# johnnyjana730/MVIN

Hardware: AMD Instinct MI355X
Metric: (user,item) pairs scored/sec @ dim=64 hop=2 fan-out=32; % HBM roofline (higher is better)
Workload: dtype f32

## Files before the change

### mvin_amd/csrc/mvin_kernels.h

```cpp
#pragma once
#include <hip/hip_runtime.h>
#include <stdint.h>

#include "../../include/mvin_hip.h"
#include "mvin_common.h"

namespace mvin {

struct GatherAttnArgs {
    int gather;
    int table_bf16;
    const void* table;
    const int32_t* adj_e;
    const int32_t* adj_r;
    const int32_t* node_ids;
    const float* neigh;
    const int32_t* rel_ids;
    const float* rel_score;
    const float* self_vec;
    const float* Wc;
    const float* c_child;
    const float* Wagg;
    const float* bagg;
    float* out;
    float* probs;
    float* s_out;
    float* z_out;
    int64_t T;
    int N, K, D, lpr_log2;
    int tile_rows;
};

struct RippleArgs {
    const void* E;
    int table_bf16;
    const int32_t* score_ids;
    const int32_t* rel_ids;
    const int32_t* value_ids;
    const float* V;
    const float* w;
    float* out;
    int64_t ldo;
    int64_t B;
    int mode, Nm, D, nR, lpr_log2;
};

struct RippleBuildArgs {
    const int64_t* indptr;
    const int32_t* dst;
    const int32_t* rel;
    const int64_t* hist_ptr;
    const int32_t* hist_items;
    int32_t* out;
    int64_t n_user;
    uint64_t seed;
    int P, Nm, n_neighbor;
};

struct KeyAddrArgs {
    const void* E;
    const float* V;
    const float* w;
    const int32_t* mem_h[8];
    const int32_t* mem_r[8];
    const int32_t* mem_t[8];
    float* out;
    int64_t ldo;
    int64_t B;
    int P, Nm, D, nR, lpr_log2;
    uint64_t table_bytes;
    const int32_t* uts;
    const int64_t* users64;
    const int32_t* users32;
    int n_user;
    int n_entity;
};

struct KeyAddrLists {
    const int32_t *h, *r, *t;
};
__device__ __forceinline__ KeyAddrLists key_addr_lists(const KeyAddrArgs& a, int64_t b, int hop) {
    if (a.uts) {
        int64_t u = a.users64 ? a.users64[b] : (int64_t)a.users32[b];
        u = u < 0 ? 0 : (u >= a.n_user ? a.n_user - 1 : u);
        const int32_t* base = a.uts + ((u * (a.P > 0 ? a.P : 1) + hop) * 3) * (int64_t)a.Nm;
        return {base, base + a.Nm, base + 2 * a.Nm};
    }
    const int64_t o = b * a.Nm;
    return {a.mem_h[hop] + o, hop < a.P ? a.mem_r[hop] + o : nullptr, hop < a.P ? a.mem_t[hop] + o : nullptr};
}

struct KeyAddrGroupedArgs {
    const void* E;
    const float* R;
    const float* w;
    const int32_t* uts;
    const int32_t* seg_user;
    const int32_t* seg_ptr;
    const int32_t* nseg_dev;
    const int32_t* pair_index;
    const int64_t* items64;
    const int32_t* items32;
    float* out;
    int64_t ldo;
    int nseg, P, Nm, D, nR, NRL;
    int n_entity;
    int dbg;
    const int32_t* records;
    const float* ER;
    const float* hs;
};

struct KaFlashArgs {
    const float* E;
    const float* ER;
    const float* hs;
    const int32_t* records;
    const int32_t* seg_user;
    const int32_t* seg_ptr;
    const int32_t* nseg_dev;
    const int32_t* pair_index;
    const int64_t* items64;
    const int32_t* items32;
    const float* TW;
    const float* bmlp;
    float* user_o;
    int32_t* slot_seg;
    int32_t* counter;
    int nslots;
    int P, Nm, nR, n_entity;
    int64_t B;
};

struct KaRecLayout {
    int NmP, rows, maxtiles, o_cnt, o_off, o_trel, o_bidx, o_head, o_tail, o_hr, len;
};

struct TailArgs {
    const void* E;
    const int64_t* items64;
    const int32_t* items32;
    const float* q;
    const float* user_o;
    const float* nagg0;
    const float* nagg1;
    const float* W0;
    const float* b0;
    const float* A0;
    const float* a0;
    const float* A1;
    const float* a1;
    const float* Wmix;
    const float* bmix;
    float* item_emb;
    float* scores;
    float* sig;
    int64_t B;
    int table_bf16;
    int n_entity;
    int dbg;
};

struct EntityAggArgs {
    const float* tabS;
    const float* tabG;
    const float* selfS;
    const float* selfG;
    const int32_t* adj_e;
    const int32_t* adj_r;
    const float* t0;
    float* outS;
    float* outG;
    int n_entity, K, nR;
    uint64_t table_bytes, adj_bytes;
    int D;
};

struct TailFoldArgs {
    const float* M0;
    const int64_t* items64;
    const int32_t* items32;
    const float* q;
    const float* user_o;
    const float* out0;
    const float* z2;
    const float* Wqm;
    const float* A1;
    const float* a1;
    const float* Wmix;
    const float* bm;
    float* item_emb;
    float* scores;
    float* sig;
    int64_t B;
    int n_entity;
};

struct GatherMixArgs {
    const void* table;
    const int32_t* adj_e;
    const int32_t* adj_r;
    const int32_t* node_ids;
    const float* rel_score;
    const float* rowbias;
    float* out;
    int64_t nodes;
    int npg, K, D, lpr_log2, relu, table_bf16;
};

struct FusedL2Args {
    const void* table;
    const int32_t* adj_e;
    const int32_t* adj_r;
    const int32_t* parent_ids;
    const float* t0;
    const float* t1;
    const float* W1;
    const float* W2;
    const float* q;
    const float* b1;
    const float* b2;
    const float* A0;
    const float* a0;
    float* nagg0;
    float* nagg1;
    float* probs_parent;
    float* probs_child;
    int64_t P;
    uint64_t table_bytes;
    uint64_t adj_bytes;
    int parents_per_pair, K, nR, lpn_log2;
    int pid_stride;
    unsigned max_id;
    int dbg;
    const int32_t* order;
    float* agg;
    int fold;
    int prj;
};

__device__ __forceinline__ int fused_parent_id(const FusedL2Args& a, int64_t i) {
    const unsigned v = (unsigned)a.parent_ids[i * a.pid_stride];
    return (int)(v < a.max_id ? v : a.max_id);
}

struct EltArgs {
    int mode;
    int64_t n;
    float* x;
    float* y;
    float* z;
    float* w;
    float* accum;
    float alpha, beta, beta1, beta2, eps;
    int D, N;
};

struct WgradArgs {
    mvin_linear_args lin;
    const float* dY;
    int64_t ldy, dy_zstride;
    const float* mask;
    int64_t ldm, mask_zstride;
    float* dW;
    int64_t dw_zstride;
    float* db;
    int64_t db_zstride;
    int IB;
};

struct AggBwdArgs {
    int gather;
    const float* table;
    const int32_t* adj_e;
    const int32_t* adj_r;
    const int32_t* node_ids;
    const float* child;
    const int32_t* rel_ids;
    const float* probs;
    const float* rel_score;
    int skip_zero;
    const float* dvec;
    float* dtable;
    float* dchild;
    float* dT;
    int64_t T;
    int K, D, nR, lpr_log2;
};

struct KeyAddrBwdArgs {
    KeyAddrArgs f;
    const float* dout;
    float* dE;
    float* dV;
    float* dw;
    float l2;
    const float* Rk;
    const void* items;
    int items64;
    int dw_rep;
    int dv_lds;
    float* reg_accum;
};

hipError_t launch_eltwise(const EltArgs& a, hipStream_t st);
hipError_t launch_l2_adam_multi(const mvin_param_seg* segs, int nseg, int64_t total, float* g, float* mo, float* vo,
                                float* accum, int apply_adam, float lr_t, const float* lr_dev, float b1, float b2,
                                float eps, hipStream_t st);
hipError_t launch_scatter_add_rows(float* dtable, const int32_t* ids, int ids64, const float* x, int64_t rows, int D,
                                   float alpha, hipStream_t st);
hipError_t launch_linear_wgrad(WgradArgs a, hipStream_t st);
hipError_t launch_linear_wgrad_multi(const WgradArgs* probs, int n, hipStream_t st);
hipError_t launch_agg_bwd(const AggBwdArgs& a, hipStream_t st);
hipError_t launch_rel_score_bwd(const float* rel, const float* urh_w, const float* dT, int nR, int D, float* drel,
                                float* durh, hipStream_t st);
hipError_t launch_key_addr_bwd(const KeyAddrBwdArgs& a, hipStream_t st);

inline int lpr_log2_for(int D) {
    int l = 0;
    while ((4 << l) < D) ++l;
    return l;
}

hipError_t launch_expand(const int32_t* adj_e, const int32_t* adj_r, const int64_t* items64,
                         const int32_t* items32, int B, int K, int levels, int n_entity,
                         int32_t* ent_out, int32_t* rel_out, hipStream_t st);
hipError_t launch_rel_score(const float* rel, const float* urh_w, int nR, int D, float* t,
                            hipStream_t st);
hipError_t launch_linear(const mvin_linear_args& a, hipStream_t st);
bool linear_mfma_supported(const mvin_linear_args& a);
hipError_t launch_linear_mfma(const mvin_linear_args& a, hipStream_t st);
hipError_t launch_gather_attn(const GatherAttnArgs& a, hipStream_t st);
hipError_t launch_ripple(const RippleArgs& a, hipStream_t st);
hipError_t launch_sample_adjacency(const int64_t* indptr, const int32_t* dst, const int32_t* rel, int n_entity,
                                   int K, uint64_t seed, int32_t* adj_e, int32_t* adj_r, hipStream_t st);
hipError_t launch_ripple_build(const RippleBuildArgs& a, hipStream_t st);
int key_addr_nj(int Nm, int D);
bool key_addr_grouped_supported(int D, int P, int Nm, int nR);
hipError_t launch_key_addr_grouped(const KeyAddrGroupedArgs& a, int table_bf16, hipStream_t st);
bool key_addr_wave16_supported(int D, int P, int Nm, int nR);
bool key_addr_wave16_applies(const KeyAddrGroupedArgs& a);
hipError_t launch_key_addr_wave16(const KeyAddrGroupedArgs& a, int table_bf16, hipStream_t st);
bool key_addr_dense_supported(int D, int P, int Nm, int nR);
hipError_t launch_key_addr_dense(const KeyAddrGroupedArgs& a, int table_bf16, hipStream_t st);
KaRecLayout ka_rec_layout(int P, int Nm, int nR);
hipError_t launch_user_records(const int32_t* uts, int n_user, int P, int Nm, int nR, int n_entity, int32_t* out, hipStream_t st);
bool key_addr_static_supported(int D, int P, int Nm, int nR);
bool key_addr_static_applies(const KeyAddrGroupedArgs& a, int table_bf16);
hipError_t launch_key_addr_static(const KeyAddrGroupedArgs& a, hipStream_t st);
bool key_addr_flash_supported(int D, int P, int Nm, int nR, int n_entity);
size_t key_addr_flash_ws_elems(int64_t B, int nseg_bound);
hipError_t launch_key_addr_flash(const KaFlashArgs& a, int nseg_bound, bool has_set, int32_t* sched_ws, hipStream_t st);
hipError_t kas_read_trace(long long* host_dst, size_t n);
hipError_t kaf_read_trace(long long* host_dst, size_t n);
hipError_t launch_key_addr(const KeyAddrArgs& a, int table_bf16, hipStream_t st);
bool key_addr_stream_supported(const KeyAddrArgs& a, int table_bf16);
hipError_t launch_key_addr_stream(const KeyAddrArgs& a, int table_bf16, hipStream_t st);
hipError_t launch_move_rows(void* table, const int32_t* ids, int64_t n, int row_bytes, void* rows, bool scatter,
                            hipStream_t st);
hipError_t launch_shard_space_ids(const void* ids, bool is64, int64_t n, int world, int n_local, void* out, hipStream_t st);
hipError_t launch_row_softmax(const float* x, int64_t rows, int n, float* out, hipStream_t st);
hipError_t launch_mix_urv(const float* neigh, const float* rel, const float* user, const float* logits, int64_t nodes, int N, int K,
                          int D, float* out, float* probs, hipStream_t st);
hipError_t launch_gather_mix(const GatherMixArgs& a, hipStream_t st);
struct ScoreSmallArgs {
    const void* E;
    const int32_t* adj_e;
    const int32_t* adj_r;
    const float* R;
    const float* w_h;
    const float* Wu;
    const float* bu;
    const float* t0;
    const float* t1;
    const float *W0, *b0, *W1, *b1, *W2, *b2;
    const float *A0, *a0, *A1, *a1, *Wmix, *bmix;
    const int64_t* items;
    const int32_t* mem_h[4];
    const int32_t* mem_r[4];
    const int32_t* mem_t[4];
    const int32_t* uts;
    const int64_t* users;
    float* user_o;
    float* item_emb;
    float* scores;
    float* sig;
    int64_t B;
    int G;
    int K, P, Nm, nR, n_entity, n_user, enc, table_bf16;
    int depth1;
    int dbg;
    uint64_t table_bytes;
    uint64_t adj_bytes;
};
bool score_small_supported(int D, int K, int P, int Nm, int nR);
int score_small_group(int D, int K, int P, int Nm, int nR, int has_hset, int64_t B);
hipError_t launch_score_small(ScoreSmallArgs a, int D, hipStream_t st);
hipError_t small_read_trace(long long* host_dst, size_t n);

bool l2_tail_supported(int D);
hipError_t launch_l2_tail(const TailArgs& a, int D, hipStream_t st);
bool l2_tail_flash_applies(const TailArgs& a, int D);
hipError_t launch_l2_tail_flash(const TailArgs& a, hipStream_t st);
bool fused_l2_supported(int D, int K);
hipError_t launch_gather_attn_l2(const FusedL2Args& a, int D, int table_bf16, hipStream_t st);
bool fused_split_supported(int D, int K);
bool fused_split_applies(const FusedL2Args& a, int D);
hipError_t launch_gather_probe_l2(const void* table, const int32_t* ids1, const int32_t* ids2, int64_t n_parents, int K,
                                  int D, int table_bf16, float* sums, hipStream_t st);
hipError_t launch_group_pairs(const int64_t* u64, const int32_t* u32, int64_t B, int n_user, int32_t* count, int32_t* offs,
                              int32_t* rank, int32_t* seg_user, int32_t* seg_ptr, int32_t* nseg, int32_t* pair_index, hipStream_t st);
hipError_t launch_count_ids(const int32_t* ids, int64_t n, int nbins, float* out, hipStream_t st);
bool fused_d32_supported(int D, int K);
bool fused_d32_applies(const FusedL2Args& a, int D);
size_t order_ws_elems(int64_t B);
hipError_t launch_order_by_key(const int64_t* k64, const int32_t* k32, int64_t B, int32_t* ws, int32_t* order, hipStream_t st);
bool fused_wpp_supported(int D, int K);
bool fused_wpp_applies(const FusedL2Args& a, int D);
hipError_t launch_gather_attn_l2_wpp(const FusedL2Args& a, hipStream_t st);
bool fused_agg_supported(int D, int K);
bool fused_fold_supported(int D, int K);
size_t fused_fold_lds_bytes(int D, int nR, int K);
bool fused_agg_applies(const FusedL2Args& a, int D);
hipError_t launch_entity_aggregates(const EntityAggArgs& a, hipStream_t st);
hipError_t launch_fold_prepare(const float* W0, const float* b0, const float* W1, const float* b1, const float* W2, const float* b2, const float* A0,
                               const float* a0, const float* Wmix, const float* bmix, const float* A1, float c, int D, float* blk, hipStream_t st);
hipError_t launch_l2_tail_fold(const TailFoldArgs& a, hipStream_t st);
hipError_t launch_score_l2_folded(const float* agg, const float* M0, const int32_t* adj_e, const int32_t* adj_r, const int32_t* items, int pid_stride,
                                  const float* t1, const float* q, const float* user_o, const float* Wq, const float* bq, const float* Wv,
                                  const float* bv, const float* Wqm, const float* A1, const float* a1, const float* Wm1, const float* Wm2,
                                  const float* bm, float* item_emb, float* scores, float* sig, int64_t B, int K, int D, int nR, int n_entity,
                                  hipStream_t st);
hipError_t launch_gather_attn_l2_agg(const FusedL2Args& a, hipStream_t st);
hipError_t launch_gather_attn_l2_d32(const FusedL2Args& a, int table_bf16, hipStream_t st, bool encoded = false);
bool fused_d16_supported(int D, int K);
bool fused_d16_applies(const FusedL2Args& a, int D);
hipError_t launch_gather_attn_l2_d16(const FusedL2Args& a, int table_bf16, hipStream_t st);
bool fused_l2_split_in_use();
hipError_t launch_gather_attn_l2_split(const FusedL2Args& a, int D, int table_bf16, hipStream_t st);
hipError_t split_read_trace(long long* host_dst, size_t n);
bool fused_packed_supported(int D, int K);
bool key_addr_static_er_ok(int P, int Nm, int nR, int n_entity, bool has_set);
hipError_t launch_transpose_blocks(const float* R, int nR, int D, float* RT, hipStream_t st);
hipError_t launch_entity_dot(const float* E, const float* w, int n, int D, float* out, hipStream_t st);
hipError_t launch_prj_prepare(const float* W1, const float* W2, const float* b1, const float* b2, const float* A0, const float* a0,
                              float c, int D, float* blk, hipStream_t st);
bool fused_packed_applies(const FusedL2Args& a, int D);
hipError_t pack_read_prof(long long* host_dst, size_t n);
hipError_t launch_gather_attn_l2_packed(const FusedL2Args& a, int D, int table_bf16, hipStream_t st);
hipError_t launch_encode_adjacency(const int32_t* adj_e, const int32_t* adj_r, int n_entity, int K, int32_t* cnt,
                                   int32_t* enc_e, int32_t* enc_r, hipStream_t st);
hipError_t ka_read_trace(long long* host_dst, size_t n);

}
```

### mvin_amd/csrc/mvin_keyaddr_flash.hip

```cpp
#include <cstdlib>
#include <type_traits>

#include "mvin_kernels.h"

namespace mvin {

typedef float f32x4 __attribute__((ext_vector_type(4)));

constexpr int kFlashChunk = 64;
constexpr int kFlashWaves = 4;

__global__ void ka_flash_slots_kernel(const int32_t* __restrict__ seg_ptr, const int32_t* __restrict__ nseg_dev, int nseg_bound,
                                      int32_t* __restrict__ slot_seg) {
    const int nseg = nseg_dev ? min(*nseg_dev, nseg_bound) : nseg_bound;
    for (int s = blockIdx.x * blockDim.x + threadIdx.x; s < nseg; s += gridDim.x * blockDim.x) {
        const int p0 = seg_ptr[s], p1 = seg_ptr[s + 1];
        const int first = p0 / kFlashChunk + s;
        const int nch = (p1 - p0 + kFlashChunk - 1) / kFlashChunk;
        for (int c = 0; c < nch; ++c) slot_seg[first + c] = s;
    }
}

#define KAF_FENCE() __builtin_amdgcn_sched_barrier(0)

__device__ long long g_kaf_trace[64 * 16];

template <int NMT, bool HAS_SET, bool TRACE = false>
__global__ __launch_bounds__(kFlashWaves * 64, 2) void key_addr_flash_kernel(KaFlashArgs a, KaRecLayout RL) {
    constexpr int D = 64;
    __shared__ f32x4 sUo0[kFlashWaves][4][64];
    const int lane = threadIdx.x & 63, l16 = lane & 15, q16 = lane >> 4;
    f32x4 (*myUo0)[64] = sUo0[threadIdx.x >> 6];
    const int P = a.P, NmP = RL.NmP;
    const unsigned emax = (unsigned)(a.n_entity - 1);
    const float* __restrict__ E = a.E;
    const size_t tw_stride = (size_t)a.n_entity * D;

    struct Rows {
        float4 v[NMT][4];
    };
    auto issue_u = [&](int mt, const int (&hr)[NMT], Rows& R) {
        const f32x4* src = reinterpret_cast<const f32x4*>(a.ER + (size_t)(unsigned)max(hr[mt], 0) * D) + q16;
#pragma unroll
        for (int nt = 0; nt < 4; ++nt) {
            const f32x4 v = __builtin_nontemporal_load(src + 4 * nt);
            R.v[mt][nt] = make_float4(v[0], v[1], v[2], v[3]);
        }
    };
    auto issue_t = [&](int mt, const float* __restrict__ tab, const int4 (&ids)[NMT], Rows& R) {
        const int id[4] = {ids[mt].x, ids[mt].y, ids[mt].z, ids[mt].w};
#pragma unroll
        for (int i = 0; i < 4; ++i)
            R.v[mt][i] = reinterpret_cast<const float4*>(tab + (size_t)(unsigned)max(id[i], 0) * D)[l16];
    };
    auto reads_tile = [&](bool two, int mt, const Rows& R, const f32x4 (&p0)[NMT], const f32x4 (&p1)[NMT], f32x4 (&u0)[4], f32x4 (&u1)[4]) {
        if (two) {
#pragma unroll
            for (int i = 0; i < 4; ++i) {
                const float t[4] = {R.v[mt][i].x, R.v[mt][i].y, R.v[mt][i].z, R.v[mt][i].w};
#pragma unroll
                for (int nt = 0; nt < 4; ++nt) u0[nt] = __builtin_amdgcn_mfma_f32_16x16x4f32(t[nt], p0[mt][i], u0[nt], 0, 0, 0);
#pragma unroll
                for (int nt = 0; nt < 4; ++nt) u1[nt] = __builtin_amdgcn_mfma_f32_16x16x4f32(t[nt], p1[mt][i], u1[nt], 0, 0, 0);
            }
        } else {
#pragma unroll
            for (int i = 0; i < 4; ++i) {
                const float t[4] = {R.v[mt][i].x, R.v[mt][i].y, R.v[mt][i].z, R.v[mt][i].w};
#pragma unroll
                for (int nt = 0; nt < 4; ++nt) u0[nt] = __builtin_amdgcn_mfma_f32_16x16x4f32(t[nt], p0[mt][i], u0[nt], 0, 0, 0);
            }
        }
    };
    auto softmax = [&](f32x4 (&lg)[NMT], const int4 (&ids)[NMT]) {
        float mx = -INFINITY;
#pragma unroll
        for (int mt = 0; mt < NMT; ++mt) {
            const int id[4] = {ids[mt].x, ids[mt].y, ids[mt].z, ids[mt].w};
#pragma unroll
            for (int i = 0; i < 4; ++i) mx = fmaxf(mx, id[i] >= 0 ? lg[mt][i] : -INFINITY);
        }
        mx = xor32_max(xor16_max(mx));
        float z = 0.f;
#pragma unroll
        for (int mt = 0; mt < NMT; ++mt) {
            const int id[4] = {ids[mt].x, ids[mt].y, ids[mt].z, ids[mt].w};
#pragma unroll
            for (int i = 0; i < 4; ++i) {
                const float x = lean_exp(fminf(lg[mt][i] - mx, 0.f));
                const float e = id[i] >= 0 ? x : 0.f;
                lg[mt][i] = e;
                z += e;
            }
        }
        z = xor32_sum(xor16_sum(z));
        const float inv = 1.f / z;
#pragma unroll
        for (int mt = 0; mt < NMT; ++mt) {
#pragma unroll
            for (int i = 0; i < 4; ++i) lg[mt][i] *= inv;
        }
    };

    int iter = 0;
    auto stamp = [&](int slot) {
        if constexpr (TRACE) {
            if (blockIdx.x == 0 && threadIdx.x == 0 && iter >= 2 && iter < 66) g_kaf_trace[(iter - 2) * 16 + slot] = __builtin_readcyclecounter();
        }
    };
    for (;; ++iter) {
        stamp(0);
        int k = 0;
        if (lane == 0) k = atomicAdd(a.counter, 1) + 1;
        k = __builtin_amdgcn_readfirstlane(k);
        if (k >= a.nslots) break;
        const int s = __builtin_amdgcn_readfirstlane(a.slot_seg[k]);
        if (s < 0) continue;
        const int u = __builtin_amdgcn_readfirstlane(a.seg_user[s]);
        const int p0 = __builtin_amdgcn_readfirstlane(a.seg_ptr[s]), p1 = __builtin_amdgcn_readfirstlane(a.seg_ptr[s + 1]);
        const int cbeg = p0 + (k - (p0 / kFlashChunk + s)) * kFlashChunk;
        const int cend = min(p1, cbeg + kFlashChunk);
        const int32_t* __restrict__ rec = a.records + (size_t)u * RL.len;
        stamp(1);
        auto load_hr = [&](int hop, int (&hr)[NMT]) {
#pragma unroll
            for (int mt = 0; mt < NMT; ++mt) hr[mt] = rec[RL.o_hr + hop * NmP + 16 * mt + l16];
        };
        auto load_tid = [&](int hop, int4 (&tid)[NMT]) {
#pragma unroll
            for (int mt = 0; mt < NMT; ++mt) tid[mt] = *reinterpret_cast<const int4*>(rec + RL.o_tail + hop * NmP + 16 * mt + 4 * q16);
        };
        auto load_orig = [&](int t0, int (&orig)[2], bool (&valid)[2]) {
#pragma unroll
            for (int rt = 0; rt < 2; ++rt) {
                const int p = t0 + 16 * rt + l16;
                valid[rt] = p < cend;
                orig[rt] = a.pair_index[min(p, cend - 1)];
            }
        };
        auto load_item = [&](const int (&orig)[2], unsigned (&item)[2]) {
#pragma unroll
            for (int rt = 0; rt < 2; ++rt)
                item[rt] = min(a.items64 ? reinterpret_cast<const unsigned*>(a.items64)[2 * (int64_t)orig[rt]] : (unsigned)a.items32[orig[rt]], emax);
        };
        auto load_be = [&](const unsigned (&item)[2], float4 (&bE)[2][4]) {
#pragma unroll
            for (int rt = 0; rt < 2; ++rt) {
#pragma unroll
                for (int nt = 0; nt < 4; ++nt) bE[rt][nt] = reinterpret_cast<const float4*>(E + (size_t)item[rt] * D)[4 * nt + q16];
            }
        };

        int orig[2], origN[2];
        bool valid[2], validN[2];
        unsigned item[2];
        float4 bE[2][4];
        int hrC[NMT], hrN[NMT];
        int4 tidC[NMT];
        Rows R;
        load_orig(cbeg, orig, valid);
        load_hr(0, hrC);
        load_tid(0, tidC);
        load_orig(cbeg + 32, origN, validN);
        f32x4 uo0[4];
#pragma unroll
        for (int r = 0; r < 4; ++r) {
            const float4 b = a.bmlp ? reinterpret_cast<const float4*>(a.bmlp)[4 * q16 + r] : make_float4(0.f, 0.f, 0.f, 0.f);
            uo0[0][r] = b.x, uo0[1][r] = b.y, uo0[2][r] = b.z, uo0[3][r] = b.w;
        }
        if constexpr (HAS_SET) {
            int4 hid[NMT];
            f32x4 ph[NMT];
#pragma unroll
            for (int mt = 0; mt < NMT; ++mt) hid[mt] = *reinterpret_cast<const int4*>(rec + RL.o_head + 16 * mt + 4 * q16);
#pragma unroll
            for (int mt = 0; mt < NMT; ++mt) issue_t(mt, a.TW, hid, R);
            KAF_FENCE();
            stamp(11);
#pragma unroll
            for (int mt = 0; mt < NMT; ++mt) {
                const int id[4] = {hid[mt].x, hid[mt].y, hid[mt].z, hid[mt].w};
#pragma unroll
                for (int i = 0; i < 4; ++i) ph[mt][i] = a.hs[max(id[i], 0)];
            }
            load_item(orig, item);
            KAF_FENCE();
            stamp(12);
            softmax(ph, hid);
            KAF_FENCE();
            stamp(13);
            f32x4 unused[4];
#pragma unroll
            for (int mt = 0; mt < NMT; ++mt) {
                reads_tile(false, mt, R, ph, ph, uo0, unused);
                KAF_FENCE();
                issue_u(mt, hrC, R);
                KAF_FENCE();
            }
            stamp(14);
        } else {
            load_item(orig, item);
#pragma unroll
            for (int mt = 0; mt < NMT; ++mt) issue_u(mt, hrC, R);
        }
        load_be(item, bE);
#pragma unroll
        for (int nt = 0; nt < 4; ++nt) myUo0[nt][lane] = uo0[nt];
        KAF_FENCE();
        stamp(2);

        const int ntile = (cend - cbeg + 31) >> 5;
        int t0 = cbeg;
        auto run_tile = [&](const bool two, const bool more) {
            f32x4 uo[2][4];
#pragma unroll
            for (int rt = 0; rt < 2; ++rt) {
#pragma unroll
                for (int nt = 0; nt < 4; ++nt) uo[rt][nt] = myUo0[nt][lane];
            }
            unsigned itemN[2];
            if (more) load_item(origN, itemN);
            for (int hop = 0; hop < P; ++hop) {
                const bool last_hop = hop + 1 == P;
                const bool next_stage = !last_hop || more;
                const int hopN = last_hop ? 0 : hop + 1;
                const float* __restrict__ tw = a.TW + (size_t)(hop + (HAS_SET ? 1 : 0)) * tw_stride;
                if (next_stage) load_hr(hopN, hrN);
                KAF_FENCE();
                if (t0 == cbeg && hop < 3) stamp(3 + 4 * hop);
                f32x4 lg[2][NMT];
#pragma unroll
                for (int mt = 0; mt < NMT; ++mt) {
                    lg[0][mt] = f32x4{0.f, 0.f, 0.f, 0.f};
                    lg[1][mt] = f32x4{0.f, 0.f, 0.f, 0.f};
                    if (two) {
#pragma unroll
                        for (int nt = 0; nt < 4; ++nt) {
                            const float av[4] = {R.v[mt][nt].x, R.v[mt][nt].y, R.v[mt][nt].z, R.v[mt][nt].w};
                            const float e0[4] = {bE[0][nt].x, bE[0][nt].y, bE[0][nt].z, bE[0][nt].w};
                            const float e1[4] = {bE[1][nt].x, bE[1][nt].y, bE[1][nt].z, bE[1][nt].w};
#pragma unroll
                            for (int i = 0; i < 4; ++i) {
                                lg[0][mt] = __builtin_amdgcn_mfma_f32_16x16x4f32(av[i], e0[i], lg[0][mt], 0, 0, 0);
                                lg[1][mt] = __builtin_amdgcn_mfma_f32_16x16x4f32(av[i], e1[i], lg[1][mt], 0, 0, 0);
                            }
                        }
                    } else {
#pragma unroll
                        for (int nt = 0; nt < 4; ++nt) {
                            const float av[4] = {R.v[mt][nt].x, R.v[mt][nt].y, R.v[mt][nt].z, R.v[mt][nt].w};
                            const float e0[4] = {bE[0][nt].x, bE[0][nt].y, bE[0][nt].z, bE[0][nt].w};
#pragma unroll
                            for (int i = 0; i < 4; ++i) lg[0][mt] = __builtin_amdgcn_mfma_f32_16x16x4f32(av[i], e0[i], lg[0][mt], 0, 0, 0);
                        }
                    }
                    KAF_FENCE();
                    issue_t(mt, tw, tidC, R);
                    KAF_FENCE();
                }
                if (last_hop && more) load_be(itemN, bE);
                KAF_FENCE();
                if (t0 == cbeg && hop < 3) stamp(4 + 4 * hop);
                softmax(lg[0], tidC);
                if (two) softmax(lg[1], tidC);
                KAF_FENCE();
                if (t0 == cbeg && hop < 3) stamp(5 + 4 * hop);
#pragma unroll
                for (int mt = 0; mt < NMT; ++mt) {
                    reads_tile(two, mt, R, lg[0], lg[1], uo[0], uo[1]);
                    KAF_FENCE();
                    if (next_stage) issue_u(mt, hrN, R);
                    KAF_FENCE();
                }
                if (next_stage) load_tid(hopN, tidC);
                if (t0 == cbeg && hop < 3) stamp(6 + 4 * hop);
            }
#pragma unroll
            for (int rt = 0; rt < 2; ++rt) {
                if (valid[rt] && (rt == 0 || two)) {
#pragma unroll
                    for (int r = 0; r < 4; ++r)
                        *reinterpret_cast<float4*>(a.user_o + (size_t)orig[rt] * D + 16 * q16 + 4 * r) =
                            make_float4(uo[rt][0][r], uo[rt][1][r], uo[rt][2][r], uo[rt][3][r]);
                }
            }
        };
        for (int tile = 0; tile < ntile; ++tile, t0 += 32) {
            const bool more = tile + 1 < ntile;
            run_tile(cend - t0 > 16, more);
#pragma unroll
            for (int rt = 0; rt < 2; ++rt) orig[rt] = origN[rt], valid[rt] = validN[rt];
        }
        stamp(15);
    }
}

hipError_t kaf_read_trace(long long* host_dst, size_t n) {
    const size_t have = sizeof(g_kaf_trace) / sizeof(long long);
    return hipMemcpyFromSymbol(host_dst, HIP_SYMBOL(g_kaf_trace), (n < have ? n : have) * sizeof(long long));
}
#undef KAF_FENCE

bool key_addr_flash_supported(int D, int P, int Nm, int nR, int n_entity) {
    if (D != 64 || P < 1 || P > 8 || Nm < 1 || Nm > 64) return false;
    const KaRecLayout RL = ka_rec_layout(P, Nm, nR);
    if (RL.len == 0) return false;
    return (long long)nR * n_entity < (1ll << 31);
}

size_t key_addr_flash_ws_elems(int64_t B, int nseg_bound) { return (size_t)(B / kFlashChunk + nseg_bound + 1) + 1; }

template <int NMT>
static hipError_t launch_flash_n(const KaFlashArgs& a, const KaRecLayout& RL, bool has_set, hipStream_t st) {
    auto k = has_set ? key_addr_flash_kernel<NMT, true> : key_addr_flash_kernel<NMT, false>;
    if constexpr (NMT == 4) {
        static const bool trace = getenv("MVIN_KAF_TRACE") != nullptr;
        if (trace && has_set) k = key_addr_flash_kernel<4, true, true>;
    }
    static thread_local int per_cu[2] = {0, 0};
    int& pc = per_cu[has_set ? 1 : 0];
    if (pc == 0) {
        int v = 0;
        if (hipOccupancyMaxActiveBlocksPerMultiprocessor(&v, reinterpret_cast<const void*>(k), kFlashWaves * 64, 0) != hipSuccess || v < 1) v = 2;
        pc = v > 8 ? 8 : v;
    }
    const int64_t want = ((int64_t)a.nslots + kFlashWaves - 1) / kFlashWaves;
    const int grid = (int)(want < 256 * (int64_t)pc ? want : 256 * (int64_t)pc);
    k<<<grid, kFlashWaves * 64, 0, st>>>(a, RL);
    return hipGetLastError();
}

hipError_t launch_key_addr_flash(const KaFlashArgs& a_, int nseg_bound, bool has_set, int32_t* sched_ws, hipStream_t st) {
    KaFlashArgs a = a_;
    const KaRecLayout RL = ka_rec_layout(a.P, a.Nm, a.nR);
    if (RL.len == 0 || !sched_ws) return hipErrorInvalidValue;
    a.nslots = (int)(a.B / kFlashChunk + nseg_bound + 1);
    a.slot_seg = sched_ws;
    a.counter = sched_ws + a.nslots;
    hipError_t e = hipMemsetAsync(sched_ws, 0xFF, ((size_t)a.nslots + 1) * sizeof(int32_t), st);
    if (e != hipSuccess) return e;
    {
        const int blocks = nseg_bound < 256 * 64 ? (nseg_bound + 255) / 256 : 64;
        ka_flash_slots_kernel<<<blocks > 0 ? blocks : 1, 256, 0, st>>>(a.seg_ptr, a.nseg_dev, nseg_bound, sched_ws);
        e = hipGetLastError();
        if (e != hipSuccess) return e;
    }
    switch (RL.NmP / 16) {
        case 1: return launch_flash_n<1>(a, RL, has_set, st);
        case 2: return launch_flash_n<2>(a, RL, has_set, st);
        case 3: return launch_flash_n<3>(a, RL, has_set, st);
        case 4: return launch_flash_n<4>(a, RL, has_set, st);
        default: return hipErrorInvalidValue;
    }
}

}
```

Measured before the change: 494.2 million.

## Compact flash slot schedule and prefetch next slot's metadata into LDS

Replaces the dense slot->segment table, which needed a full memset to -1 and produced empty slots, with a compact schedule. Each segment's first chunk maps directly to its own slot index, and only extra chunks are appended through an atomic list. Each wave double-buffers the next slot's descriptor, hop-0 record indices, pair indices and items in LDS (items through global_load_lds), so these latency-bound loads overlap with current compute. Bias is cached in LDS. The cost is more LDS use, which could lower occupancy, plus extra control complexity.

```diff
diff --git a/mvin_amd/csrc/mvin_kernels.h b/mvin_amd/csrc/mvin_kernels.h
--- a/mvin_amd/csrc/mvin_kernels.h
+++ b/mvin_amd/csrc/mvin_kernels.h
@@ -125,9 +125,9 @@
     const float* TW;
     const float* bmlp;
     float* user_o;
-    int32_t* slot_seg;
-    int32_t* counter;
-    int nslots;
+    int32_t* sched;
+    int nseg_bound;
+    int extra_cap;
     int P, Nm, nR, n_entity;
     int64_t B;
 };
diff --git a/mvin_amd/csrc/mvin_keyaddr_flash.hip b/mvin_amd/csrc/mvin_keyaddr_flash.hip
--- a/mvin_amd/csrc/mvin_keyaddr_flash.hip
+++ b/mvin_amd/csrc/mvin_keyaddr_flash.hip
@@ -9,15 +9,22 @@
 
 constexpr int kFlashChunk = 64;
 constexpr int kFlashWaves = 4;
-
-__global__ void ka_flash_slots_kernel(const int32_t* __restrict__ seg_ptr, const int32_t* __restrict__ nseg_dev, int nseg_bound,
-                                      int32_t* __restrict__ slot_seg) {
+constexpr int kStHead = 0, kStHr = 64, kStTail = 128, kStPair = 192, kStItem = 256, kStDesc = 320, kStWords = 324;
+
+__global__ void ka_flash_slots_kernel(const int32_t* __restrict__ seg_user, const int32_t* __restrict__ seg_ptr,
+                                      const int32_t* __restrict__ nseg_dev, int nseg_bound, int extra_cap, int32_t* __restrict__ sched) {
     const int nseg = nseg_dev ? min(*nseg_dev, nseg_bound) : nseg_bound;
     for (int s = blockIdx.x * blockDim.x + threadIdx.x; s < nseg; s += gridDim.x * blockDim.x) {
         const int p0 = seg_ptr[s], p1 = seg_ptr[s + 1];
-        const int first = p0 / kFlashChunk + s;
-        const int nch = (p1 - p0 + kFlashChunk - 1) / kFlashChunk;
-        for (int c = 0; c < nch; ++c) slot_seg[first + c] = s;
+        const int nex = (p1 - p0 - 1) / kFlashChunk;
+        if (nex <= 0) continue;
+        const int u = seg_user[s];
+        const int first = p0 + ((p1 - p0 - 1) & (kFlashChunk - 1)) + 1;
+        const int j = atomicAdd(sched + 1, nex);
+        for (int c = 0; c < nex && j + c < extra_cap; ++c) {
+            sched[2 + 2 * (j + c)] = u;
+            sched[3 + 2 * (j + c)] = first + c * kFlashChunk;
+        }
     }
 }
 
@@ -31,6 +38,10 @@
     __shared__ f32x4 sUo0[kFlashWaves][4][64];
     const int lane = threadIdx.x & 63, l16 = lane & 15, q16 = lane >> 4;
     f32x4 (*myUo0)[64] = sUo0[threadIdx.x >> 6];
+    __shared__ int sStage[kFlashWaves][2][kStWords];
+    int (*myStage)[kStWords] = sStage[threadIdx.x >> 6];
+    __shared__ float sBias[kFlashWaves][64];
+    float* myBias = sBias[threadIdx.x >> 6];
     const int P = a.P, NmP = RL.NmP;
     const unsigned emax = (unsigned)(a.n_entity - 1);
     const float* __restrict__ E = a.E;
@@ -108,40 +119,114 @@
             if (blockIdx.x == 0 && threadIdx.x == 0 && iter >= 2 && iter < 66) g_kaf_trace[(iter - 2) * 16 + slot] = __builtin_readcyclecounter();
         }
     };
+    myBias[lane] = a.bmlp ? a.bmlp[lane] : 0.f;
+    const int nseg = a.nseg_dev ? min(__builtin_amdgcn_readfirstlane(*a.nseg_dev), a.nseg_bound) : a.nseg_bound;
+    const int n_extra = min(__builtin_amdgcn_readfirstlane(a.sched[1]), a.extra_cap);
+    const int nslots = n_extra + nseg;
+    auto draw_issue = [&]() -> int {
+        int k = 0;
+        if (lane == 0) k = (int)atomicInc(reinterpret_cast<unsigned*>(a.sched), 0xFFFFFFFFu);
+        return k;
+    };
+    auto draw_take = [&](int k) { return __builtin_amdgcn_readfirstlane(k); };
+    struct Slot {
+        int u, cbeg, cend;
+    };
+    auto describe_issue = [&](int k) -> int {
+        if (k >= nslots) return 0;
+        const int32_t* src;
+        if (k < n_extra) {
+            src = a.sched + 2 + 2 * k + (lane == 1 ? 1 : 0);
+        } else {
+            const int s = k - n_extra;
+            src = lane == 1 ? a.seg_ptr + s : lane == 2 ? a.seg_ptr + s + 1 : a.seg_user + s;
+        }
+        return *src;
+    };
+    auto slot_of = [&](int k, int v) -> Slot {
+        Slot d{0, 0, 0};
+        if (k >= nslots) return d;
+        d.u = __builtin_amdgcn_readlane(v, 0);
+        d.cbeg = __builtin_amdgcn_readlane(v, 1);
+        d.cend = k < n_extra ? d.cbeg + kFlashChunk : d.cbeg + ((__builtin_amdgcn_readlane(v, 2) - d.cbeg - 1) & (kFlashChunk - 1)) + 1;
+        return d;
+    };
+    auto describe = [&](int k) -> Slot { return slot_of(k, describe_issue(k)); };
+    const int li = lane < NmP ? lane : 0;
+    struct StageRegs {
+        int head, hr, tail, pair;
+    };
+    auto stage_load = [&](const Slot& d) -> StageRegs {
+        const int32_t* __restrict__ r = a.records + (size_t)d.u * RL.len;
+        StageRegs g;
+        g.head = HAS_SET ? r[RL.o_head + li] : 0;
+        g.hr = r[RL.o_hr + li];
+        g.tail = r[RL.o_tail + li];
+        g.pair = a.pair_index[min(d.cbeg + lane, d.cend - 1)];
+        return g;
+    };
+    auto stage_write = [&](int* st, const StageRegs& g) {
+        if constexpr (HAS_SET) st[kStHead + lane] = g.head;
+        st[kStHr + lane] = g.hr;
+        st[kStTail + lane] = g.tail;
+        st[kStPair + lane] = g.pair;
+    };
+    const unsigned* __restrict__ items = a.items64 ? reinterpret_cast<const unsigned*>(a.items64) : reinterpret_cast<const unsigned*>(a.items32);
+    const int item_shift = a.items64 ? 1 : 0;
+    auto item_stage = [&](int* st, int pair) {
+        __builtin_amdgcn_global_load_lds((__attribute__((address_space(1))) const void*)(items + ((int64_t)pair << item_shift)),
+                                         (__attribute__((address_space(3))) void*)(st + kStItem), 4, 0, 0);
+    };
+    auto desc_write = [&](int* st, const Slot& d) {
+        if (lane < 3) st[kStDesc + lane] = lane == 0 ? d.u : lane == 1 ? d.cbeg : d.cend;
+    };
+    auto desc_read = [&](const int* st) -> Slot {
+        return Slot{__builtin_amdgcn_readfirstlane(st[kStDesc]), __builtin_amdgcn_readfirstlane(st[kStDesc + 1]),
+                    __builtin_amdgcn_readfirstlane(st[kStDesc + 2])};
+    };
+
+    int kc = draw_take(draw_issue());
+    const Slot dc = describe(kc);
+    if (kc < nslots) {
+        const StageRegs g = stage_load(dc);
+        stage_write(myStage[0], g);
+        desc_write(myStage[0], dc);
+        item_stage(myStage[0], g.pair);
+    }
+    int kn = kc < nslots ? draw_take(draw_issue()) : nslots;
+    Slot dn = describe(kn);
+    int cur = 0;
+
     for (;; ++iter) {
+        if (kc >= nslots) break;
         stamp(0);
-        int k = 0;
-        if (lane == 0) k = atomicAdd(a.counter, 1) + 1;
-        k = __builtin_amdgcn_readfirstlane(k);
-        if (k >= a.nslots) break;
-        const int s = __builtin_amdgcn_readfirstlane(a.slot_seg[k]);
-        if (s < 0) continue;
-        const int u = __builtin_amdgcn_readfirstlane(a.seg_user[s]);
-        const int p0 = __builtin_amdgcn_readfirstlane(a.seg_ptr[s]), p1 = __builtin_amdgcn_readfirstlane(a.seg_ptr[s + 1]);
-        const int cbeg = p0 + (k - (p0 / kFlashChunk + s)) * kFlashChunk;
-        const int cend = min(p1, cbeg + kFlashChunk);
+        const int nxt = cur ^ 1;
+        const bool has_next = kn < nslots;
+        const Slot dc = desc_read(myStage[cur]);
+        const int u = dc.u, cbeg = dc.cbeg, cend = dc.cend;
         const int32_t* __restrict__ rec = a.records + (size_t)u * RL.len;
-        stamp(1);
+        const int* __restrict__ st = myStage[cur];
         auto load_hr = [&](int hop, int (&hr)[NMT]) {
 #pragma unroll
-            for (int mt = 0; mt < NMT; ++mt) hr[mt] = rec[RL.o_hr + hop * NmP + 16 * mt + l16];
+            for (int mt = 0; mt < NMT; ++mt) hr[mt] = hop == 0 ? st[kStHr + 16 * mt + l16] : rec[RL.o_hr + hop * NmP + 16 * mt + l16];
         };
         auto load_tid = [&](int hop, int4 (&tid)[NMT]) {
 #pragma unroll
-            for (int mt = 0; mt < NMT; ++mt) tid[mt] = *reinterpret_cast<const int4*>(rec + RL.o_tail + hop * NmP + 16 * mt + 4 * q16);
-        };
-        auto load_orig = [&](int t0, int (&orig)[2], bool (&valid)[2]) {
+            for (int mt = 0; mt < NMT; ++mt)
+                tid[mt] = hop == 0 ? *reinterpret_cast<const int4*>(st + kStTail + 16 * mt + 4 * q16)
+                                   : *reinterpret_cast<const int4*>(rec + RL.o_tail + hop * NmP + 16 * mt + 4 * q16);
+        };
+        auto load_orig = [&](int tile, int (&orig)[2], bool (&valid)[2]) {
 #pragma unroll
             for (int rt = 0; rt < 2; ++rt) {
-                const int p = t0 + 16 * rt + l16;
-                valid[rt] = p < cend;
-                orig[rt] = a.pair_index[min(p, cend - 1)];
-            }
-        };
-        auto load_item = [&](const int (&orig)[2], unsigned (&item)[2]) {
-#pragma unroll
-            for (int rt = 0; rt < 2; ++rt)
-                item[rt] = min(a.items64 ? reinterpret_cast<const unsigned*>(a.items64)[2 * (int64_t)orig[rt]] : (unsigned)a.items32[orig[rt]], emax);
+                const int i = 32 * tile + 16 * rt + l16;
+                valid[rt] = cbeg + i < cend;
+                orig[rt] = st[kStPair + i];
+            }
+        };
+        auto load_item = [&](int tile, unsigned (&item)[2]) {
+#pragma unroll
+            for (int rt = 0; rt < 2; ++rt) item[rt] = min((unsigned)st[kStItem + 32 * tile + 16 * rt + l16], emax);
         };
         auto load_be = [&](const unsigned (&item)[2], float4 (&bE)[2][4]) {
 #pragma unroll
@@ -158,21 +243,34 @@
         int hrC[NMT], hrN[NMT];
         int4 tidC[NMT];
         Rows R;
-        load_orig(cbeg, orig, valid);
+        load_orig(0, orig, valid);
         load_hr(0, hrC);
         load_tid(0, tidC);
-        load_orig(cbeg + 32, origN, validN);
+        load_orig(1, origN, validN);
+        load_item(0, item);
+        int4 hid[NMT];
+        if constexpr (HAS_SET) {
+#pragma unroll
+            for (int mt = 0; mt < NMT; ++mt) hid[mt] = *reinterpret_cast<const int4*>(st + kStHead + 16 * mt + 4 * q16);
+        }
+        KAF_FENCE();
+        stamp(1);
+        StageRegs gN{0, 0, 0, 0};
+        int kv = 0;
+        if (has_next) {
+            gN = stage_load(dn);
+            kv = draw_issue();
+            desc_write(myStage[nxt], dn);
+        }
+        KAF_FENCE();
         f32x4 uo0[4];
 #pragma unroll
         for (int r = 0; r < 4; ++r) {
-            const float4 b = a.bmlp ? reinterpret_cast<const float4*>(a.bmlp)[4 * q16 + r] : make_float4(0.f, 0.f, 0.f, 0.f);
+            const float4 b = reinterpret_cast<const float4*>(myBias)[4 * q16 + r];
             uo0[0][r] = b.x, uo0[1][r] = b.y, uo0[2][r] = b.z, uo0[3][r] = b.w;
         }
         if constexpr (HAS_SET) {
-            int4 hid[NMT];
             f32x4 ph[NMT];
-#pragma unroll
-            for (int mt = 0; mt < NMT; ++mt) hid[mt] = *reinterpret_cast<const int4*>(rec + RL.o_head + 16 * mt + 4 * q16);
 #pragma unroll
             for (int mt = 0; mt < NMT; ++mt) issue_t(mt, a.TW, hid, R);
             KAF_FENCE();
@@ -183,7 +281,6 @@
 #pragma unroll
                 for (int i = 0; i < 4; ++i) ph[mt][i] = a.hs[max(id[i], 0)];
             }
-            load_item(orig, item);
             KAF_FENCE();
             stamp(12);
             softmax(ph, hid);
@@ -199,13 +296,20 @@
             }
             stamp(14);
         } else {
-            load_item(orig, item);
 #pragma unroll
             for (int mt = 0; mt < NMT; ++mt) issue_u(mt, hrC, R);
         }
         load_be(item, bE);
 #pragma unroll
         for (int nt = 0; nt < 4; ++nt) myUo0[nt][lane] = uo0[nt];
+        KAF_FENCE();
+        int kf = nslots;
+        if (has_next) {
+            stage_write(myStage[nxt], gN);
+            item_stage(myStage[nxt], gN.pair);
+            kf = draw_take(kv);
+        }
+        const int dv = describe_issue(kf);
         KAF_FENCE();
         stamp(2);
 
@@ -219,7 +323,7 @@
                 for (int nt = 0; nt < 4; ++nt) uo[rt][nt] = myUo0[nt][lane];
             }
             unsigned itemN[2];
-            if (more) load_item(origN, itemN);
+            if (more) load_item(1, itemN);
             for (int hop = 0; hop < P; ++hop) {
                 const bool last_hop = hop + 1 == P;
                 const bool next_stage = !last_hop || more;
@@ -292,6 +396,7 @@
             for (int rt = 0; rt < 2; ++rt) orig[rt] = origN[rt], valid[rt] = validN[rt];
         }
         stamp(15);
+        kc = kn, kn = kf, dn = slot_of(kf, dv), cur = nxt;
     }
 }
 
@@ -308,7 +413,11 @@
     return (long long)nR * n_entity < (1ll << 31);
 }
 
-size_t key_addr_flash_ws_elems(int64_t B, int nseg_bound) { return (size_t)(B / kFlashChunk + nseg_bound + 1) + 1; }
+static int flash_extra_cap(int64_t B) { return (int)((B - 1) / kFlashChunk); }
+size_t key_addr_flash_ws_elems(int64_t B, int nseg_bound) {
+    (void)nseg_bound;
+    return 2 + 2 * (size_t)flash_extra_cap(B);
+}
 
 template <int NMT>
 static hipError_t launch_flash_n(const KaFlashArgs& a, const KaRecLayout& RL, bool has_set, hipStream_t st) {
@@ -324,7 +433,7 @@
         if (hipOccupancyMaxActiveBlocksPerMultiprocessor(&v, reinterpret_cast<const void*>(k), kFlashWaves * 64, 0) != hipSuccess || v < 1) v = 2;
         pc = v > 8 ? 8 : v;
     }
-    const int64_t want = ((int64_t)a.nslots + kFlashWaves - 1) / kFlashWaves;
+    const int64_t want = ((int64_t)a.nseg_bound + a.extra_cap + kFlashWaves - 1) / kFlashWaves;
     const int grid = (int)(want < 256 * (int64_t)pc ? want : 256 * (int64_t)pc);
     k<<<grid, kFlashWaves * 64, 0, st>>>(a, RL);
     return hipGetLastError();
@@ -334,14 +443,15 @@
     KaFlashArgs a = a_;
     const KaRecLayout RL = ka_rec_layout(a.P, a.Nm, a.nR);
     if (RL.len == 0 || !sched_ws) return hipErrorInvalidValue;
-    a.nslots = (int)(a.B / kFlashChunk + nseg_bound + 1);
-    a.slot_seg = sched_ws;
-    a.counter = sched_ws + a.nslots;
-    hipError_t e = hipMemsetAsync(sched_ws, 0xFF, ((size_t)a.nslots + 1) * sizeof(int32_t), st);
+    if (a.B < 1) return hipErrorInvalidValue;
+    a.sched = sched_ws;
+    a.nseg_bound = nseg_bound;
+    a.extra_cap = flash_extra_cap(a.B);
+    hipError_t e = hipMemsetAsync(sched_ws, 0, 2 * sizeof(int32_t), st);
     if (e != hipSuccess) return e;
     {
         const int blocks = nseg_bound < 256 * 64 ? (nseg_bound + 255) / 256 : 64;
-        ka_flash_slots_kernel<<<blocks > 0 ? blocks : 1, 256, 0, st>>>(a.seg_ptr, a.nseg_dev, nseg_bound, sched_ws);
+        ka_flash_slots_kernel<<<blocks > 0 ? blocks : 1, 256, 0, st>>>(a.seg_user, a.seg_ptr, a.nseg_dev, nseg_bound, a.extra_cap, sched_ws);
         e = hipGetLastError();
         if (e != hipSuccess) return e;
     }
```

After: 499.9 million, median of 6. +1.2%, better.
